# neofytr/LLMTokenizer

Measured on AMD Instinct MI355X. Metric: corpus MB/s per merge iter (train), 1 GiB synthetic corpus, higher is better.
Workload: dtype u32

## Files before the change

include/bpe_gpu.h:

```cpp
#ifndef BPE_GPU_H
#define BPE_GPU_H

#include <stddef.h>
#include <stdint.h>

#ifdef __cplusplus
extern "C" {
#endif

enum {
    BPE_GPU_OK = 0,
    BPE_GPU_EINVAL = -1,
    BPE_GPU_EHIP = -2,
    BPE_GPU_ENOMEM = -3,
    BPE_GPU_ENODEV = -4,
    BPE_GPU_ESTATE = -5,
    BPE_GPU_ERANGE = -6,
    BPE_GPU_EDATA = -7,
    BPE_GPU_EINTERNAL = -8,
    BPE_GPU_EIO = -9
};

typedef struct bpe_gpu_ctx bpe_gpu_ctx;

// ... 109 lines not shown
int bpe_gpu_decode_docs(bpe_gpu_ctx *ctx, const uint32_t *ids, size_t len, const uint64_t *id_off,
                        size_t ndocs, const uint32_t *pairs, size_t n_merges,
                        uint8_t *out, size_t cap, size_t *out_len, uint64_t *byte_off);
int bpe_gpu_docs_window(const uint64_t *doc_off, size_t ndocs, uint64_t n,
                        uint32_t core, uint32_t halo, uint64_t w, uint64_t *out8);

enum { BPE_SPLIT_LINES = 0, BPE_SPLIT_WORDS = 1 };
#define BPE_GPU_SPLIT_TILE 4096
#define BPE_GPU_SPLIT_GRID 2048
int bpe_gpu_split_rule(int preset, uint8_t *cls, uint16_t *brk);
int bpe_gpu_split_info(uint64_t *out4);
int bpe_gpu_split(bpe_gpu_ctx *ctx, const uint8_t *cls, const uint16_t *brk, size_t *ndocs);
int bpe_gpu_fetch_split_offsets(bpe_gpu_ctx *ctx, uint64_t *out, size_t cap, size_t *count);
int bpe_gpu_encode_split(bpe_gpu_ctx *ctx, const uint32_t *pairs, size_t n_merges);

int bpe_gpu_get_stats(bpe_gpu_ctx *ctx, bpe_gpu_stats *st);

int bpe_gpu_ids_checksum(bpe_gpu_ctx *ctx, uint64_t base, uint64_t *sum);

int bpe_gpu_device_tokens(bpe_gpu_ctx *ctx, const void **dev_tok, size_t *n);

int bpe_gpu_set_profile(bpe_gpu_ctx *ctx, int on);

int bpe_gpu_kernel_profile(bpe_gpu_ctx *ctx, const char **name, double *avg_ms,
                           double *bytes_per_launch, uint64_t *launches);

int bpe_gpu_event_profile(bpe_gpu_ctx *ctx, double *avg_ms, uint64_t *launches);

#define BPE_GPU_P2P_HANDLE_BYTES 64
#define BPE_GPU_P2P_MAX_RANKS 16
// ... 35 lines not shown
```

llmtokenizer_amd/_lib.py:

```python
import atexit
import ctypes
import os

HERE = os.path.dirname(os.path.abspath(__file__))
LIB_PATH = os.environ.get("BPE_LIB") or os.path.join(HERE, "libbpe_amd.so")

EXPORTS = [
    "get_file", "dump_pairs", "read_pairs", "print_text", "print_graph", "compress",
    "decompress", "render_pairs", "resolve_pair", "is_less",
    "dyn_arr_create", "dyn_arr_free", "dyn_arr_set", "dyn_arr_append", "dyn_arr_get",
    "dyn_arr_sort", "dyn_arr_max", "dyn_arr_min",
    "hash_table_create", "hash_table_destroy", "hash_table_insert", "hash_table_delete",
    "hash_table_search", "hash_table_clear", "hash_table_merge",
    "compress_ex", "bpe_train_bytes", "bpe_encode_bytes", "bpe_last_stats",
    "bpe_train_bytes_devices", "compress_multi", "bpe_release_engines", "bpe_encode_docs", "bpe_decode_docs",
    "bpe_encode_split",
    "bpe_gpu_device_count", "bpe_gpu_create", "bpe_gpu_destroy", "bpe_gpu_load", "bpe_gpu_synth",
    "bpe_gpu_train", "bpe_gpu_fetch_merges", "bpe_gpu_fetch_ids", "bpe_gpu_encode", "bpe_gpu_decode",
    "bpe_gpu_get_stats", "bpe_gpu_set_merge_log", "bpe_gpu_fetch_merge_log", "bpe_gpu_device_tokens", "bpe_gpu_kernel_profile", "bpe_gpu_set_profile", "bpe_gpu_event_profile",
    "bpe_gpu_strerror",
    "bpe_gpu_last_error", "bpe_gpu_train_ex",
    "bpe_gpu_comm_id", "bpe_gpu_group_create", "bpe_gpu_group_destroy", "bpe_gpu_group_shards",
    "bpe_gpu_group_load", "bpe_gpu_group_synth", "bpe_gpu_group_train", "bpe_gpu_group_encode", "bpe_gpu_group_fetch_merges",
    "bpe_gpu_group_fetch_ids", "bpe_gpu_group_get_stats", "bpe_gpu_group_exchange_mode", "bpe_gpu_shard_halo", "bpe_gpu_group_kernel_profile",
    "bpe_gpu_group_create_p2p", "bpe_gpu_group_p2p_connect", "bpe_gpu_group_transport",
    "bpe_gpu_group_create_local_p2p", "bpe_gpu_ids_checksum", "bpe_gpu_group_ids_checksum", "bpe_gpu_load_fd",
    "bpe_gpu_fetch_ids_range", "bpe_gpu_group_fetch_ids_range", "bpe_gpu_device_pci", "bpe_gpu_peer_access",
    "bpe_gpu_fetch_events", "bpe_gpu_trim",
    "bpe_gpu_encode_docs", "bpe_gpu_fetch_doc_offsets", "bpe_gpu_docs_info", "bpe_gpu_decode_docs",
    "bpe_gpu_docs_window",
    "bpe_gpu_split_rule", "bpe_gpu_split_info", "bpe_gpu_split", "bpe_gpu_fetch_split_offsets", "bpe_gpu_encode_split",
]


class GpuStats(ctypes.Structure):
    _fields_ = [(n, ctypes.c_uint64) for n in (
        "n_in", "n_out", "merges", "iterations", "distinct_pairs", "merged_buckets",
        "tracked_iters", "tie_events", "edge_events", "rule_ties", "table_grows", "keys")] + \
        [(n, ctypes.c_double) for n in ("ms_init", "ms_train", "ms_total", "ms_count_pass")] + \
        [(n, ctypes.c_uint64) for n in ("candidates", "occurrences", "l1_rescanned", "spec_hits", "spec_misses",
                                                     "count_pass_span", "hot_rebuilds", "hot_mode", "hot_scanned",
                                                     "enc_path", "enc_windows", "relists", "batches",
                                                     "batch_dropped", "batch_retries", "table_updates")] + \
        [(n, ctypes.c_double) for n in ("ms_scan_span", "ms_apply_span")] + \
        [(n, ctypes.c_uint64) for n in ("track_exact", "track_skipped", "track_violations", "track_light")] + \
        [(n, ctypes.c_uint64) for n in ("end_list", "end_count", "end_skipgate", "end_dup", "end_tie", "end_conflict",
# ... 120 lines not shown
    L.bpe_gpu_fetch_doc_offsets.argtypes = [vp, vp, sz, ctypes.POINTER(sz)]
    L.bpe_gpu_docs_info.argtypes = [vp, vp]
    L.bpe_gpu_decode_docs.argtypes = [vp, vp, sz, vp, sz, vp, sz, vp, sz, ctypes.POINTER(sz), vp]
    L.bpe_gpu_docs_window.argtypes = [vp, sz, ctypes.c_uint64, ctypes.c_uint32, ctypes.c_uint32, ctypes.c_uint64, vp]
    L.bpe_encode_docs.argtypes = [vp, sz, vp, sz, ctypes.POINTER(DynArr), ctypes.c_int, ctypes.POINTER(sz),
                                  ctypes.POINTER(u64p)]
    L.bpe_encode_docs.restype = u32p
    L.bpe_decode_docs.argtypes = [vp, sz, vp, sz, ctypes.POINTER(DynArr), ctypes.c_int, ctypes.POINTER(sz),
                                  ctypes.POINTER(u64p)]
    L.bpe_decode_docs.restype = ctypes.c_void_p
    L.bpe_gpu_split_rule.argtypes = [ctypes.c_int, vp, vp]
    L.bpe_gpu_split_info.argtypes = [vp]
    L.bpe_gpu_split.argtypes = [vp, vp, vp, ctypes.POINTER(sz)]
    L.bpe_gpu_fetch_split_offsets.argtypes = [vp, vp, sz, ctypes.POINTER(sz)]
    L.bpe_gpu_encode_split.argtypes = [vp, vp, sz]
    L.bpe_encode_split.argtypes = [vp, sz, vp, vp, ctypes.POINTER(DynArr), ctypes.c_int, ctypes.POINTER(sz),
                                   ctypes.POINTER(u64p), ctypes.POINTER(u64p), ctypes.POINTER(sz)]
    L.bpe_encode_split.restype = u32p
    L.bpe_release_engines.argtypes = []
    L.bpe_release_engines.restype = None
    _LIB = L
    atexit.register(L.bpe_release_engines)
    return L


def check(rc, what):
    if rc != 0:
        L = load()
        raise BpeError(f"{what}: {L.bpe_gpu_strerror(rc).decode()} ({L.bpe_gpu_last_error().decode()})")
```

llmtokenizer_amd/api.py:

```python
import ctypes
import os
import weakref

import numpy as np

from . import _lib
from ._lib import BpeError, GpuStats

_u32p = ctypes.POINTER(ctypes.c_uint32)


def _arr_to_merges(arr_p):
    L = _lib.load()
    last = arr_p.contents.last_index
    k = max(0, last - 255)
    out = np.zeros((k, 2), dtype=np.uint32)
    buf = (ctypes.c_uint32 * 2)()
    for r in range(k):
        if not L.dyn_arr_get(arr_p, 256 + r, ctypes.cast(buf, ctypes.c_void_p)):
            raise BpeError(f"merge list has no record for id {256 + r}")
        out[r] = (buf[0], buf[1])
    return out


# ... 129 lines not shown
def split_rule(preset):
    if preset not in SPLIT_PRESETS:
        raise BpeError(f"split_rule: no preset {preset!r} (have {sorted(SPLIT_PRESETS)})")
    L = _lib.load()
    cls = np.zeros(256, dtype=np.uint8)
    brk = np.zeros(16, dtype=np.uint16)
    _lib.check(L.bpe_gpu_split_rule(SPLIT_PRESETS[preset], cls.ctypes.data_as(ctypes.c_void_p),
                                    brk.ctypes.data_as(ctypes.c_void_p)), "split_rule")
    return cls, brk


def split_info():
    out = np.zeros(4, dtype=np.uint64)
    _lib.check(_lib.load().bpe_gpu_split_info(out.ctypes.data_as(ctypes.c_void_p)), "split_info")
    return {"tile": int(out[0]), "grid_bytes": int(out[1])}


def _rule_tables(rule):
    cls, brk = split_rule(rule) if isinstance(rule, str) else rule
    cls = np.ascontiguousarray(cls, dtype=np.uint8).reshape(-1)
    brk = np.ascontiguousarray(brk, dtype=np.uint16).reshape(-1)
    if cls.size != 256 or brk.size != 16:
        raise BpeError("split rule: cls must hold 256 entries and brk 16")
    return cls, brk


def encode_split(data: bytes, merges, rule="words", device=0):
    L = _lib.load()
    cls, brk = _rule_tables(rule)
    buf = np.frombuffer(data, dtype=np.uint8)
# ... 433 lines not shown
```

llmtokenizer_amd/csrc/batch.hip:

```cpp
#pragma once
#include "engine_common.h"

namespace bpeamd {

static_assert(TOPK == 64, "a wave holds a list, one entry per lane");
static_assert(BRB == 2 * (1024 / 64), "the select's 16 waves merge two partial lists each");
#ifndef BPE_SU
#define BPE_SU 1
#endif
#ifndef BPE_FORM_PRINT
#define BPE_FORM_PRINT 0
#endif
#ifndef BPE_RU
#define BPE_RU 4
#endif
#ifndef BPE_AU
#define BPE_AU 1
#endif
constexpr uint32_t AU = BPE_AU;
constexpr uint32_t SU = BPE_SU;
#ifndef BPE_RUN_THREAD_PAIRS
#define BPE_RUN_THREAD_PAIRS 16
#endif
constexpr uint32_t RUN_THREAD_PAIRS = BPE_RUN_THREAD_PAIRS, RUN_Q = 256;
// ... 29 lines not shown
        const uint32_t c = (uint32_t)__popcll(lo);
        if (r >= c) {
            r -= c;
            M >>= w;
            pos += w;
        } else {
            M = lo;
        }
    }
    return pos;
}

enum { BT_SCAN_IN = 0, BT_SCAN_CAND, BT_SCAN_OUT, BT_APPLY_IN, BT_APPLY_PRO, BT_APPLY_A, BT_APPLY_B, BT_SEL_IN,
       BT_SEL_RED, BT_SEL_LIST, BT_SEL_OUT, BT_SEL_FORMED, BT_SEL_CAND, BT_SEL_FOLD, BT_SEL_WB,
       BT_F_TIE, BT_F_CM, BT_F_MEMB, BT_F_FOLD, BT_F_PRE, BT_F_CHK, BT_B_DEC, BT_B_UPD, BT_R_LOAD, BT_R_SORT, BT_R_TREE, BT_N };
static_assert(BT_N <= TS_N, "batch stamps fit a timeline row");
__device__ inline uint32_t bat_idx(const Eng *E) {
    return E->dbgts ? (uint32_t)(E->bat->nbatch + E->bat->nretry) : 0u;
}

struct KV {
    unsigned long long v, k;
};
__device__ __attribute__((always_inline)) inline KV kv_empty() { return KV{0ull, ~0ull}; }
__device__ __attribute__((always_inline)) inline bool kv_ahead(const KV &x, const KV &y) { return x.v > y.v || (x.v == y.v && x.k < y.k); }
__device__ __attribute__((always_inline)) inline KV kv_shfl(const KV &x, int src) { return KV{__shfl(x.v, src), __shfl(x.k, src)}; }
__device__ __attribute__((always_inline)) inline KV kv_xor(const KV &x, int m) { return KV{__shfl_xor(x.v, m), __shfl_xor(x.k, m)}; }

__device__ __attribute__((always_inline)) inline KV wave_sort64(KV x) {
    const uint32_t lane = lane_id();
#pragma unroll
// ... 583 lines not shown
            prev = kv_shfl(ep, 63);
            __builtin_amdgcn_fence(__ATOMIC_RELEASE, "wavefront");
            __builtin_amdgcn_wave_barrier();
            if (!more) break;
        }
    }
    }
    uint32_t k = kk;
    if (tid < 64 && stop == STOP_NONE) {
        ts_mark(E, bi, BT_SEL_FORMED, false);
#if BPE_FORM_PRINT
        if (E->dbg_form && md + 1 >= E->dbg_form && lane == 0)
            printf("form shard %u md %u passes %u k %u end %u why %u skipped %u D %llu B %llu pend %u zrate %u\n", E->shard,
                   md, npass, kk, kend, endwhy, nskt, D, (unsigned long long)Bsz, tpend, B->zrate);
#endif
        uint32_t mode[NBK], off[NBK], len[NBK], tl[NBK], slot[NBK], slot_k[NBK], nb[NBK], bpre[NBK];
        unsigned long long pre[NBK];
#pragma unroll
        for (uint32_t b = 0; b < NBK; b++) {
            const uint32_t q = 64 * b + lane;
            mode[b] = 1;
            off[b] = len[b] = tl[b] = 0;
            if (q < k) {
                const uint32_t mu = fm_u[q], mv = fm_v[q];
                cand_of(E, mu, mv, true, srank, E->poff, &mode[b], &off[b], &len[b]);
                const uint32_t tlu = E->tlen[mu], tlv = E->tlen[mv];
                tl[b] = tlu + tlv;
                Bg->mla[q] = tlu;
                Bg->mlb[q] = tlv;
                Bg->nskb[q] = (uint8_t)fm_nsk[q];
                Bg->cnew[q] = 0;
// ... 15 lines not shown
            why_end = 7;
        }
        const unsigned long long pcut = sh && ovm < k ? bank_shfl(pre, ovm - 1) : 0ull;
        unsigned long long sumlen = 0;
#pragma unroll
        for (uint32_t b = 0; b < NBK; b++) {
            const uint32_t q = 64 * b + lane;
            slot_k[b] = slot[b];
            if (sh && q >= ovm) len[b] = slot_k[b] = 0;
            if (sh && ovm < k && q >= ovm) pre[b] = pcut;
            sumlen += q < k ? len[b] : 0u;
        }
        const unsigned long long stage_end = bank_shfl(pre, k - 1);
        sumlen = wave_sum(sumlen);
        uint32_t wk[NBK];
        unsigned long long sumw = 0, big = 0;
#pragma unroll
        for (uint32_t b = 0; b < NBK; b++) {
            const uint32_t q = 64 * b + lane;
            wk[b] = q < k && mode[b] != 0 && E->scan_occd ? min(len[b], fm_c[q] + len[b] / E->scan_occd) : len[b];
            sumw += q < k ? wk[b] : 0u;
        }
        sumw = wave_sum(sumw);
#pragma unroll
        for (uint32_t b = 0; b < NBK; b++) {
            const uint32_t q = 64 * b + lane;
            nb[b] = q < k ? 1 + (uint32_t)(sumw ? (uint64_t)(BSB - k) * wk[b] / sumw : 0) : 0;
            bpre[b] = nb[b];
            if (q < k) big = max(big, ((unsigned long long)wk[b] << 8) | (255u - q));
        }
        bank_scan(bpre);
        for (int o = 32; o > 0; o >>= 1) big = max(big, (unsigned long long)__shfl_xor(big, o));
        const uint32_t used = bank_shfl(bpre, k - 1);
        const uint32_t bigm = 255u - (uint32_t)(big & 255u);
        const uint32_t extra = BSB - used;
#pragma unroll
        for (uint32_t b = 0; b < NBK; b++) {
            const uint32_t q = 64 * b + lane;
            if (q < k) {
                B->a[q] = fm_u[q];
                B->b[q] = fm_v[q];
                B->cnt[q] = fm_c[q];
                B->mode[q] = mode[b];
                B->off[q] = off[b];
                B->len[q] = len[b];
                B->sbase[q] = (uint32_t)(pre[b] - slot_k[b]);
                B->R[q] = 0;
                B->bound[q] = 0;
                B->blk0[q] = bpre[b] - nb[b] + (q > bigm ? extra : 0);
                B->tmask[q] = (uint8_t)fm_tm[q];
                B->tspan[q] = (uint32_t)min(fm_span[q], 0xFFFFFFFFull);
                ctl[q] = tl[b];
            }
        }
        const uint32_t nsk = k ? fm_nsk[k - 1] : 0u;
        if (lane == 0) {
            B->sbase[k] = (uint32_t)stage_end;
            B->blk0[k] = BSB;
            B->sumlen = (uint32_t)sumlen;
            B->over = ovm < k ? ovm : BK;
            B->tpend = tpend < k ? tpend : BK;
            Bg->nsk = nsk;
            Bg->gr_n = 0;
#pragma unroll
            for (uint32_t g = 0; g < GRUN; g++) {
                Bg->gr_tk[g] = 0;
                Bg->gr_endc[g] = 0xFFFFFFFFu;
                Bg->gr_ready[g] = 0;
            }
            B->ztot = 0;
            B->tbar = 0;
            B->tlog_n = 0;
            B->why[why_end]++;
// ... 547 lines not shown
            }
#pragma unroll
            for (uint32_t bb = 0; bb < NBK; bb++) {
                unsigned long long tm = tadj.w[bb];
                for (int o = 32; o > 0; o >>= 1) tm |= __shfl_xor(tm, o);
                if (lane == 0 && tm) atomicOr(&B->adj[mg][bb], tm);
            }
        }
    }
}

template <bool SH>
__global__ __launch_bounds__(SCAN_T) void k_bscan(const Eng *__restrict__ E, const Ctl *__restrict__ C) {
    if (C->stop) return;
    Bat *B = E->bat;
    const uint32_t bi = bat_idx(E);
    ts_mark(E, bi, BT_SCAN_IN, true);
    if (threadIdx.x == 0) atomicMax(&B->sc_in, ~wall_clock64());
    __shared__ uint32_t s[4][DENSE];
    __shared__ uint32_t list[SCAN_T * SU * FR];
    __shared__ uint16_t ltag[SCAN_T * SU * FR];
    __shared__ uint32_t lcount, gbase, list_n, covc, sm, sk, sz0, bRs;
    __shared__ uint32_t lr_n, lr_brk, lr_pos[RUN_Q];
    __shared__ unsigned long long badj[NBK];
    __shared__ uint32_t gcnt[2];
    __shared__ uint32_t sa[BK], sb[BK];
    __shared__ RoleTab rt;
    __shared__ BHalo H;
    __shared__ uint32_t wmx[2][16];
    const uint32_t tid = threadIdx.x;
    const uint32_t sgen = ((uint32_t)(B->nbatch + B->nretry) & 0x0FFFFFFFu) + 1u;
    if (tid == 0) {
        sm = BK;
        covc = lcount = bRs = 0;
        lr_n = 0;
#pragma unroll
        for (uint32_t b = 0; b < NBK; b++) badj[b] = 0;
        gcnt[0] = gcnt[1] = 0;
        sk = B->k;
        sz0 = B->z0;
    }
    for (uint32_t q = tid; q < RH; q += SCAN_T) {
        rt.id[q] = HOLE;
        rt.fl[q] = 0;
    }
    for (uint32_t q = tid; q < RP; q += SCAN_T) rt.pk[q] = 0;
    uint32_t mla = 0;
    if (tid < BK) {
        const uint32_t lo = B->blk0[tid], hi = B->blk0[tid + 1];
        const uint32_t ma = B->a[tid];
        sa[tid] = ma;
        sb[tid] = B->b[tid];
        mla = E->tlen[ma];
        if (blockIdx.x >= lo && blockIdx.x < hi && tid < B->k) sm = tid;
    }
    __syncthreads();
    const uint32_t k = sk, m = sm, z0 = sz0;
    if (m >= k) {
        if (tid == 0) atomicMax(&B->sc_out, wall_clock64());
        return;
    }
    MK tadj = mk_zero();
    if (tid < k) {
        rt.put(sa[tid], sb[tid], mla, tid);
        if (SH) {
            Halo h;
            shard_halo(E->erec, E->nshards, E->shard, sa[tid], &h);
            H.hlr[tid] = h.hlrun;
            H.myi[tid] = h.myidx;
            if (tid == 0)
                for (int q = 0; q < 3; q++) {
                    H.HL[q] = h.HL[q];
                    H.HR[q] = h.HR[q];
                }
        }
    }
    const uint32_t a = sa[m], b = sb[m], z = z0 + m;
    const uint32_t la = E->tlen[a], lb = E->tlen[b];
    const uint32_t mode = B->mode[m], off = B->off[m], len = B->len[m];
    const uint32_t bid = blockIdx.x - B->blk0[m], nblk = B->blk0[m + 1] - B->blk0[m];
    const uint32_t sbase = B->sbase[m];
    uint32_t *occz = E->ids_out + sbase;
    uint16_t *tagz = E->btag + sbase;
    const uint32_t sslice = B->sbase[m + 1] - sbase;
#define STG(IDX, WHERE) if ((IDX) >= sslice) { B->ra_err = 12; } else
    uint32_t *Rm = &B->R[m];
    const int64_t n = (int64_t)E->n0;
    const uint32_t *__restrict__ tok = E->tok;
    const uint32_t want = mode == 2 ? a : b;
    const uint32_t lim = min(DENSE, z0 + k);
    for (uint32_t v = 0; v < 4; v++)
        for (uint32_t x = tid; x < lim; x += SCAN_T) s[v][x] = 0;
    __syncthreads();
    auto tok_at = [&](int64_t p) -> uint32_t { return tok_at_b<SH>(tok, H, p, n); };

    if (a != b) {
        static_assert(SU == 1 && BPE_WFLUSH, "the wave-driven candidate loop: one entry per lane per round");
        const uint32_t stride = nblk * SCAN_T;
        const uint32_t lane = tid & 63, wbase = (tid >> 6) * 64 * FR;
        uint32_t wcnt = 0, wocc = 0;
        uint32_t nent[SU];
        uint16_t ntg[SU];
        uint32_t eS = bid * SCAN_T + (tid & ~63u);
        auto load1 = [&](uint32_t s0, uint32_t &en, uint16_t &tg) {
            const uint32_t e = s0 + lane;
            en = 0;
            tg = 0xFFFFu;
            if (e < len) {
                en = mode == 0 ? E->plist[off + e] : E->occ[off + e];
                if (mode) tg = E->occnb[off + e];
            }
        };
        uint32_t pent = 0;
        uint16_t ptg = 0xFFFFu;
        auto advance = [&]() {
            eS += stride;
            if (SCAN_PD > 1) {
                nent[0] = pent;
// ... 12 lines not shown
            for (uint32_t q = lane; q < wcnt; q += 64) {
                STG(g + q, "wflush") {
                occz[g + q] = list[wbase + q];
                tagz[g + q] = ltag[wbase + q];
                }
            }
            wocc += wcnt;
            wcnt = 0;
            __builtin_amdgcn_wave_barrier();
        };
        const bool cmp = mode != 0 && E->scan_compact != 0;
        const uint32_t tsh = mode == 2 ? 8u : 0u;
        uint32_t qpos = 0, qn = 0;
        load1(eS, nent[0], ntg[0]);
        if (SCAN_PD > 1) load1(eS + stride, pent, ptg);
        for (;;) {
            uint32_t ent[SU];
            uint16_t etg[SU];
            bool val[SU];
            if (!cmp) {
                if (eS >= len) break;
                val[0] = eS + lane < len;
                ent[0] = nent[0];
                etg[0] = ntg[0];
                advance();
            } else {
                while (eS < len) {
                    const bool pass = eS + lane < len && tag_ok(((uint32_t)ntg[0] >> tsh) & 0xFFu, want);
                    const unsigned long long M = __ballot(pass);
                    const uint32_t np = (uint32_t)__popcll(M);
                    if (qn + np > 64) break;
                    const uint32_t r = lane - qn;
                    const bool mine = lane >= qn && r < np;
                    const uint32_t pv = (uint32_t)__shfl((int)nent[0], (int)(mine ? kth_bit(M, r) : lane));
                    if (mine) qpos = pv;
                    qn += np;
                    advance();
                }
                if (qn == 0) break;
                val[0] = lane < qn;
                ent[0] = qpos;
                etg[0] = 0xFFFFu;
                qn = 0;
            }
            int64_t ii[SU], jj[SU];
            TokWin W[SU];
#pragma unroll
            for (uint32_t u = 0; u < SU; u++) {
                if (mode == 2) {
                    val[u] = val[u] && tag_ok(etg[u] >> 8, want);
                    jj[u] = ent[u];
                    ii[u] = 0;
                    if (val[u]) W[u] = tok_window(tok, jj[u]);
                } else {
                    val[u] = val[u] && (mode == 0 || tag_ok(etg[u] & 0xFFu, want));
                    ii[u] = ent[u];
                    jj[u] = ii[u] + la;
                    if (val[u]) W[u] = tok_window(tok, ii[u]);
                }
            }
            bool ok[SU];
// ... 62 lines not shown
                    }
                }
                const unsigned long long om = __ballot(ok[u]);
                if (ok[u]) {
                    const uint32_t slot = wbase + wcnt + (uint32_t)__popcll(om & ((1ull << lane) - 1ull));
                    list[slot] = (uint32_t)i;
                    ltag[slot] = nb_tag(lfin, rfin);
                }
                wcnt += (uint32_t)__popcll(om);
            }
            if (wcnt + 64 > 64 * FR) flush();
        }
        if (wcnt) flush();
        if (lane == 0 && wocc) atomicAdd(&bRs, wocc);
    } else {
        for (uint32_t e0 = bid * SCAN_T; e0 < len; e0 += nblk * SCAN_T) {
            const uint32_t e = e0 + tid;
            int64_t i = 0;
            bool ok = false;
            if (e >= len) {
            } else if (mode == 2) {
                const int64_t j = E->occ[off + e];
                if (tag_ok(E->occnb[off + e] >> 8, want) && tok[j] == b) {
                    i = v_left<SH>(tok, j);
                    ok = i >= 0 && tok[i] == a;
                }
            } else {
                i = (mode == 0) ? E->plist[off + e] : E->occ[off + e];
                ok = (mode == 0 || tag_ok(E->occnb[off + e] & 0xFFu, want)) && tok[i] == a && i + la < n &&
                     tok[i + la] == b;
            }
// ... 63 lines not shown
                const uint32_t c = min(lcount, SCAN_T * SU);
                gbase = c ? atomicAdd(Rm, c) : 0u;
                bRs += c;
                lcount = 0;
                list_n = c;
            }
            __syncthreads();
            for (uint32_t q = tid; q < list_n; q += SCAN_T) {
                STG(gbase + q, "tflush") {
                occz[gbase + q] = list[q];
                tagz[gbase + q] = ltag[q];
                }
            }
            __syncthreads();
        }
        const uint32_t lane = tid & 63, wv = tid >> 6, nlr = min(lr_n, RUN_Q);
        auto segs = [&](int64_t c, uint32_t o, auto Uc, auto &&live) -> bool {
            constexpr uint32_t U = decltype(Uc)::value;
            const int64_t L0 = (n - c + la - 1) / la;
            auto posl = [&](int64_t l) -> int64_t { return l < L0 ? c + l * la : n + (l - L0); };
            int64_t P[U];
            uint32_t t[U], tx[U], f[U];
#pragma unroll
            for (uint32_t u = 0; u < U; u++) {
                const int64_t ou = (int64_t)o + 64 * u;
                P[u] = posl(ou + lane);
                t[u] = tok_at(P[u]);
                tx[u] = lane < 2 ? tok_at(posl(ou + 64 + lane)) : HOLE;
            }
            uint32_t fb = U;
#pragma unroll
// ... 57 lines not shown
                    segs(c, 64 * RUN_BU * wv, std::integral_constant<uint32_t, RUN_BU>{}, [&](uint32_t fb) {
                        if (lane == 0 && fb < RUN_BU) atomicMin(&lr_brk, wv * RUN_BU + fb);
                        __syncthreads();
                        const uint32_t gb = lr_brk, w0 = wv * RUN_BU;
                        return gb < w0 ? 0u : min(RUN_BU, gb - w0 + 1);
                    });
                    const bool done = lr_brk < NS;
                    __syncthreads();
                    if (done) break;
                    c += (int64_t)NS * 64 * la;
                }
            }
        }
    }
    __syncthreads();
    if (!SH && E->grflag) bscan_long_runs(E, B, tok, rt, H, n, z0, sgen);
    ts_mark(E, bi, BT_SCAN_CAND, false, true);
    if (tid < SKMAX && tid < B->nsk && ((B->sk_cm[tid][m >> 6] >> (m & 63)) & 1ull)) {
        const uint32_t xs = B->sk_a[tid], ys = B->sk_b[tid];
        uint32_t d = 0;
        if (xs == b && ys < lim) d += s[V_DR][ys];
        if (ys == a && xs < lim) d += s[V_DL][xs];
        if (d) atomicAdd(SH ? &E->xbat[BK + tid] : &B->sdec[tid], d);
    }
    const uint32_t Wx = xbat_vw(z0 + k);
    uint32_t *xm = SH ? E->xbat + XBH + (uint64_t)m * xbat_member_words(Wx) : nullptr;
    if (SH && blockIdx.x == 0 && tid == 0) {
        uint32_t xlm = BK;
        const int64_t F1 = C->F1, L1 = C->L1;
        const uint32_t over = B->over;
        if (F1 < n) {
            const uint32_t tf = tok[F1], tl1 = tok[L1];
            for (uint32_t mm = 0; mm < k; mm++)
                if (H.HL[0] == sa[mm] && tf == sb[mm] && (sa[mm] != sb[mm] || (H.hlr[mm] & 1))) {
                    xlm = mm;
                    break;
                }
            for (uint32_t mm = 0; mm < k && mm < over; mm++) {
                if (!(tl1 == sa[mm] && H.HR[0] == sb[mm] && (sa[mm] != sb[mm] || !(H.myi[mm] & 1)))) continue;
                uint32_t *xo = E->xbat + XBH + (uint64_t)mm * xbat_member_words(Wx);
                const uint32_t zz = z0 + mm;
// ... 17 lines not shown
                    if (st < BK) rfin = z0 + st;
                    xadd(E, xo, Wx, mm, V_DR, q);
                    xadd(E, xo, Wx, mm, V_IR, rfin);
                }
                (void)zz;
                const uint32_t g = atomicAdd(&B->R[mm], 1u);
                E->ids_out[B->sbase[mm] + g] = (uint32_t)L1;
                E->btag[B->sbase[mm] + g] = nb_tag(lfin, rfin);
                atomicAdd(&xo[0], 1u);
                atomicAdd(&xo[1], bnd);
                break;
            }
        }
        B->xl_m = xlm;
        if (over < k) atomicAdd(&E->xbat[over], 1u);
    }
    if (k > 1) {
#pragma unroll
        for (uint32_t bb = 0; bb < NBK; bb++) {
            unsigned long long t = tadj.w[bb];
            for (int o = 32; o > 0; o >>= 1) t |= __shfl_xor(t, o);
            if ((tid & 63) == 0 && t) atomicOr(&badj[bb], t);
        }
        __syncthreads();
        if (tid < NBK && badj[tid]) atomicOr(&B->adj[m][tid], badj[tid]);
    }
    uint32_t *rep = SH ? xm + 2 : E->bvecd + (uint64_t)(m * BREPL + bid % BREPL) * 4 * DENSE;
    const uint32_t vstride = SH ? Wx : DENSE;
    uint32_t mxl = 0, mxr = 0;
    for (uint32_t v = 0; v < 4; v++)
        for (uint32_t x = tid; x < lim; x += SCAN_T) {
            const uint32_t c = s[v][x];
            if (c) atomicAdd(&rep[v * vstride + x], c);
            if (v == V_DL) mxl = max(mxl, c);
            if (v == V_DR) mxr = max(mxr, c);
        }
    if (SH && tid == 0 && bRs) atomicAdd(&xm[0], bRs);
    if (k > 1) {
        for (int o = 32; o > 0; o >>= 1) {
            mxl = max(mxl, (uint32_t)__shfl_xor(mxl, o));
            mxr = max(mxr, (uint32_t)__shfl_xor(mxr, o));
        }
        if ((tid & 63) == 0) {
            wmx[0][tid >> 6] = mxl;
            wmx[1][tid >> 6] = mxr;
        }
        __syncthreads();
        if (tid == 0) {
            uint32_t l = 0, r = 0;
            for (uint32_t q = 0; q < SCAN_T / 64; q++) {
                l = max(l, wmx[0][q]);
                r = max(r, wmx[1][q]);
            }
            atomicAdd(SH ? &xm[1] : &B->bound[m], max(l + gcnt[V_DL] + covc, r + gcnt[V_DR]));
        }
    }
    ts_mark(E, bi, BT_SCAN_OUT, false, true);
    asm volatile("s_waitcnt vmcnt(0)" ::: "memory");
    __syncthreads();
    if (tid == 0) atomicMax(&B->sc_out, wall_clock64());
}
template __global__ void k_bscan<false>(const Eng *, const Ctl *);
template __global__ void k_bscan<true>(const Eng *, const Ctl *);

constexpr uint32_t XSP_SHIFT = 23;
static_assert(4 * BK < (1u << (32 - XSP_SHIFT)), "member-vector index fits above the id");
__global__ __launch_bounds__(256) void k_bpack(const Eng *__restrict__ E, const Ctl *__restrict__ C) {
    if (C->stop) return;
    const Bat *B = E->bat;
    __shared__ uint32_t pre[BK * 4 + 1];
// ... 660 lines not shown
```

llmtokenizer_amd/csrc/engine.hip:

```cpp
#include <hip/hip_runtime.h>
#include <fcntl.h>
#include <unistd.h>
#include <cerrno>

#include <algorithm>
#include <chrono>
#include <cstdio>
#include <cstdlib>
#include <cstring>
#include <string>
#include <thread>
#include <vector>
#include <unordered_map>

#include <rocprim/rocprim.hpp>

#include "../../include/bpe_gpu.h"
#include "kernels.hip"
#include "batch.hip"
#include "encode.hip"
#include "encode_win.hip"
#include "encode_docs.hip"
#include "split.hip"

// ... 1418 lines not shown
        const unsigned long long *r = &t[(size_t)b * TS_N];
        bool ok = true;
        for (int k = 0; k < BT_N; k++) ok = ok && r[k] != 0;
        if (!ok) continue;
        const double t0 = (double)~r[BT_SCAN_IN];
        for (int k = 0; k < BT_N; k++) {
            const bool in = k == BT_SCAN_IN || k == BT_APPLY_IN || k == BT_SEL_IN;
            sum[k] += ((in ? (double)~r[k] : (double)r[k]) - t0) * 1000.0 / khz;
        }
        n++;
        const unsigned long long *q = &t[(size_t)(b + 1) * TS_N];
        if (q[BT_SCAN_IN]) {
            gap += ((double)~q[BT_SCAN_IN] - (double)r[BT_SEL_OUT]) * 1000.0 / khz;
            ng++;
        }
    }
    if (!n) return;
    fprintf(stderr, "batch timeline over %u batches (us from k_bscan's first block entry):", n);
    for (int k = 1; k < BT_N; k++) fprintf(stderr, " %s %.2f;", nm[k], sum[k] / n);
    fprintf(stderr, " sel out -> next scan in %.2f\n", ng ? gap / ng : 0.0);
}

int batch_stats(bpe_gpu_ctx *c) {
    if (!c->h.bat) return 0;
    Bat hb;
    HIPCHK(hipMemcpy(&hb, c->h.bat, offsetof(Bat, pv), hipMemcpyDeviceToHost));
    c->stats.batches = hb.nbatch;
    c->stats.batch_dropped = hb.ndrop;
    c->stats.batch_retries = hb.nretry;
    c->stats.table_updates = hb.nupd;
// ... 1571 lines not shown
                 : b >= '\t' && b <= '\r'                                      ? 4
                                                                               : 0;
    for (int p = 0; p < 5; p++) brk[p] = (uint16_t)(0x1F & ~(1 << p));
    brk[3] = 1 << 4;
    return 0;
}

int bpe_gpu_split_info(uint64_t *out4) {
    if (!out4) return BPE_GPU_EINVAL;
    out4[0] = SP_TILE;
    out4[1] = (uint64_t)SP_TILE * SP_GRID;
    out4[2] = out4[3] = 0;
    return 0;
}

int bpe_gpu_split(bpe_gpu_ctx *c, const uint8_t *cls, const uint16_t *brk, size_t *ndocs) {
    if (!c || !cls || !brk || !ndocs) return BPE_GPU_EINVAL;
    if (!c->loaded) return fail(BPE_GPU_ESTATE, "split before load");
    SplitRule R;
    for (int b = 0; b < 256; b++)
        if ((R.cls[b] = cls[b]) > 15) return fail(BPE_GPU_EINVAL, "split: a class above 15");
    memcpy(R.brk, brk, sizeof R.brk);
    HIPCHK(hipSetDevice(c->dev));
    c->split_ready = false;
    const uint64_t n = c->n0, ntiles = (n + SP_TILE - 1) / SP_TILE, nwt = ntiles * (SP_T / 64);
    unsigned long long total = 0;
    uint16_t *mask = nullptr;
    unsigned long long *woff = nullptr;
    int r;
    if (n) {
// ... 107 lines not shown
```

llmtokenizer_amd/csrc/engine_common.h:

```cpp
#pragma once
#include <hip/hip_runtime.h>
#include <stddef.h>
#include <stdint.h>

namespace bpeamd {

constexpr uint32_t HOLE = 0xFFFFFFFFu;
constexpr uint32_t END_FLAG = 0x80000000u;
constexpr uint32_t MARKV = 0xFFFFFFFEu;
constexpr uint64_t END_MAX = 0x7FFFFFFDull;
__host__ __device__ inline bool is_id(uint32_t v) { return v < END_FLAG; }
__host__ __device__ inline uint32_t end_code(uint64_t d) { return END_FLAG | (uint32_t)d; }
#ifndef BPE_DENSE
#define BPE_DENSE 8192
#endif
constexpr uint32_t DENSE = BPE_DENSE;
#ifndef BPE_REPL
#define BPE_REPL 8
#endif
constexpr uint32_t REPL = BPE_REPL;
constexpr uint32_t NTHR = 16;
constexpr uint64_t CHUNK = 65536;
constexpr uint64_t DYN_LIMIT = CHUNK * NTHR;
constexpr uint64_t TRACK_LIMIT = 2 * DYN_LIMIT;
constexpr uint64_t TRACK_MIN_N = 4096;
constexpr uint64_t MERGED_B0 = 65536;
constexpr uint64_t THREAD_B0 = 256;
constexpr uint32_t L1W = 1024;
constexpr uint32_t L2W = 256;
constexpr uint32_t EDGE_WORDS = 16;
constexpr uint32_t TS_SLOTS = 16384;
enum { TS_K1_IN = 0, TS_K1_RESCAN, TS_K1_SCAN, TS_K2_IN, TS_K2_SELECT, TS_K2_APPLY_A, TS_K2_APPLY_B, TS_K1_LASTIN,
       TS_S_CAND, TS_S_LIST, TS_S_DELTA, TS_B_DVAL, TS_B_TABLE, TS_B_MARKS, TS_B_PROBE, TS_B_COUNT, TS_K1_CLEARED,
       TS_SPARE0, TS_SPARE1, TS_SPARE2, TS_SPARE3, TS_SPARE4, TS_SPARE5, TS_SPARE6, TS_SPARE7, TS_SPARE8, TS_N };

enum { V_DL = 0, V_DR = 1, V_IL = 2, V_IR = 3 };

enum : uint32_t {
    STOP_NONE = 0,
    STOP_DONE = 1,
    STOP_CAP = 2,
    STOP_EVENT = 3,
    STOP_GROW = 4,
    STOP_ERROR = 5,
    STOP_ENC_END = 6,
    STOP_MODE = 7,
    STOP_REDO = 8,
    STOP_HOT = 9,
    STOP_RELIST = 10,
// ... 35 lines not shown
constexpr uint32_t TOPK = 64;
#ifndef BPE_BK
#define BPE_BK 127
#endif
constexpr uint32_t BK = BPE_BK;
constexpr uint32_t NBK = (BK + 1) / 64;
static_assert(BK + 1 == 64 * NBK && NBK >= 1 && NBK <= 2, "BK is 63 or 127");
constexpr uint32_t SKMAX = BK;
#ifndef BPE_NLIST
#define BPE_NLIST 4
#endif
constexpr uint32_t NLIST = BPE_NLIST;
constexpr uint32_t BRB = 32;
constexpr uint32_t BREPL = 2;
constexpr uint32_t BSB = 256;
constexpr uint32_t STALL_LIMIT = 64;
constexpr uint32_t GRUN = 4;
constexpr uint32_t GR_CH = 16384;
constexpr uint32_t GR_PROBE = 4096;
__host__ __device__ inline uint64_t gr_stride(uint64_t n0) { return n0 / GR_CH + 2; }
constexpr uint32_t P2P_MAXR_B = 16;

struct Bat {
    uint32_t k, z0, applied, jstar;
    uint32_t ticket, retry, sumlen, rhold;
    unsigned long long dD;
    unsigned long long nbatch, ndrop, nretry;
    unsigned long long why[8];
    uint32_t drop_test;
    uint32_t skgate;
    unsigned long long stage_cap;
    unsigned long long sc_in, sc_out, ap_in, ap_out, sc_ticks, ap_ticks, nspan, nupd;
    uint32_t a[BK], b[BK], cnt[BK], mode[BK], off[BK], len[BK];
    uint32_t blk0[BK + 1];
    uint32_t sbase[BK + 1];
    uint32_t R[BK];
    uint32_t bound[BK];
    uint32_t Rg[BK];
    uint32_t over;
    uint32_t xl_m;
    uint32_t tpend;
    uint32_t ztot;
    uint32_t tbar, zrate;
    unsigned long long ntie, ntfail, nzero;
    uint8_t tmask[BK + 1];
    uint32_t tspan[BK];
    uint32_t tlog_n;
    unsigned long long pv[BRB * TOPK], pk[BRB * TOPK];
    uint32_t ra_k, ra_top, ra_done, ra_err;
// ... 323 lines not shown
```

Measured before the change: 118.7 million.

## Split batch scan work across blocks by weighted granules instead of whole merges

The old scheme gave each batched merge a whole number of k_bscan blocks, sized by its share of the weight plus leftovers assigned to the largest merge. The new scheme takes a prefix sum of per-merge weights and cuts the global weighted range into equal slices of 1024-entry granules, so one block can cover the tail of one merge and the head of later ones. The scan body now loops over those pieces with per-piece reset and flush of the shared histograms. The intent is to balance load across the 256 blocks and avoid a single overloaded block. The cost is more flushes and syncthreads per block, plus extra debug busy-time counters and a host-side test API.

```diff
diff --git a/include/bpe_gpu.h b/include/bpe_gpu.h
--- a/include/bpe_gpu.h
+++ b/include/bpe_gpu.h
@@ -147,6 +147,9 @@
 int bpe_gpu_fetch_split_offsets(bpe_gpu_ctx *ctx, uint64_t *out, size_t cap, size_t *count);
 int bpe_gpu_encode_split(bpe_gpu_ctx *ctx, const uint32_t *pairs, size_t n_merges);
 
+int bpe_gpu_scan_split(const uint32_t *weight, const uint32_t *len, uint32_t k, uint32_t nblk, uint32_t block,
+                       uint32_t *pieces, size_t cap, size_t *count);
+
 int bpe_gpu_get_stats(bpe_gpu_ctx *ctx, bpe_gpu_stats *st);
 
 int bpe_gpu_ids_checksum(bpe_gpu_ctx *ctx, uint64_t base, uint64_t *sum);
diff --git a/llmtokenizer_amd/_lib.py b/llmtokenizer_amd/_lib.py
--- a/llmtokenizer_amd/_lib.py
+++ b/llmtokenizer_amd/_lib.py
@@ -30,6 +30,7 @@
     "bpe_gpu_encode_docs", "bpe_gpu_fetch_doc_offsets", "bpe_gpu_docs_info", "bpe_gpu_decode_docs",
     "bpe_gpu_docs_window",
     "bpe_gpu_split_rule", "bpe_gpu_split_info", "bpe_gpu_split", "bpe_gpu_fetch_split_offsets", "bpe_gpu_encode_split",
+    "bpe_gpu_scan_split",
 ]
 
 
@@ -180,6 +181,7 @@
     L.bpe_gpu_split.argtypes = [vp, vp, vp, ctypes.POINTER(sz)]
     L.bpe_gpu_fetch_split_offsets.argtypes = [vp, vp, sz, ctypes.POINTER(sz)]
     L.bpe_gpu_encode_split.argtypes = [vp, vp, sz]
+    L.bpe_gpu_scan_split.argtypes = [vp, vp, ctypes.c_uint32, ctypes.c_uint32, ctypes.c_uint32, vp, sz, ctypes.POINTER(sz)]
     L.bpe_encode_split.argtypes = [vp, sz, vp, vp, ctypes.POINTER(DynArr), ctypes.c_int, ctypes.POINTER(sz),
                                    ctypes.POINTER(u64p), ctypes.POINTER(u64p), ctypes.POINTER(sz)]
     L.bpe_encode_split.restype = u32p
diff --git a/llmtokenizer_amd/api.py b/llmtokenizer_amd/api.py
--- a/llmtokenizer_amd/api.py
+++ b/llmtokenizer_amd/api.py
@@ -167,6 +167,19 @@
     out = np.zeros(4, dtype=np.uint64)
     _lib.check(_lib.load().bpe_gpu_split_info(out.ctypes.data_as(ctypes.c_void_p)), "split_info")
     return {"tile": int(out[0]), "grid_bytes": int(out[1])}
+
+
+def scan_split(weight, length, nblk, block):
+    w = np.ascontiguousarray(weight, dtype=np.uint32).reshape(-1)
+    n = np.ascontiguousarray(length, dtype=np.uint32).reshape(-1)
+    if w.size != n.size:
+        raise BpeError("scan_split: one weight per list")
+    out = np.zeros((max(1, w.size), 3), dtype=np.uint32)
+    cnt = ctypes.c_size_t(0)
+    _lib.check(_lib.load().bpe_gpu_scan_split(w.ctypes.data_as(ctypes.c_void_p), n.ctypes.data_as(ctypes.c_void_p),
+                                              w.size, nblk, block, out.ctypes.data_as(ctypes.c_void_p),
+                                              out.shape[0], ctypes.byref(cnt)), "scan_split")
+    return [tuple(int(x) for x in row) for row in out[:cnt.value]]
 
 
 def _rule_tables(rule):
diff --git a/llmtokenizer_amd/csrc/batch.hip b/llmtokenizer_amd/csrc/batch.hip
--- a/llmtokenizer_amd/csrc/batch.hip
+++ b/llmtokenizer_amd/csrc/batch.hip
@@ -67,7 +67,9 @@
 enum { BT_SCAN_IN = 0, BT_SCAN_CAND, BT_SCAN_OUT, BT_APPLY_IN, BT_APPLY_PRO, BT_APPLY_A, BT_APPLY_B, BT_SEL_IN,
        BT_SEL_RED, BT_SEL_LIST, BT_SEL_OUT, BT_SEL_FORMED, BT_SEL_CAND, BT_SEL_FOLD, BT_SEL_WB,
        BT_F_TIE, BT_F_CM, BT_F_MEMB, BT_F_FOLD, BT_F_PRE, BT_F_CHK, BT_B_DEC, BT_B_UPD, BT_R_LOAD, BT_R_SORT, BT_R_TREE, BT_N };
-static_assert(BT_N <= TS_N, "batch stamps fit a timeline row");
+enum { BT_X_BUSY_SUM = TS_X0, BT_X_BUSY_MAX = TS_X1, BT_X_BUSY_N = TS_X2 };
+static_assert(BT_N <= TS_X0, "batch stamps fit a timeline row");
+static_assert(SCAN_GRAN == 1024, "a granule is one round of a k_bscan block");
 __device__ inline uint32_t bat_idx(const Eng *E) {
     return E->dbgts ? (uint32_t)(E->bat->nbatch + E->bat->nretry) : 0u;
 }
@@ -681,7 +683,7 @@
             printf("form shard %u md %u passes %u k %u end %u why %u skipped %u D %llu B %llu pend %u zrate %u\n", E->shard,
                    md, npass, kk, kend, endwhy, nskt, D, (unsigned long long)Bsz, tpend, B->zrate);
 #endif
-        uint32_t mode[NBK], off[NBK], len[NBK], tl[NBK], slot[NBK], slot_k[NBK], nb[NBK], bpre[NBK];
+        uint32_t mode[NBK], off[NBK], len[NBK], tl[NBK], slot[NBK], slot_k[NBK], wpre[NBK];
         unsigned long long pre[NBK];
 #pragma unroll
         for (uint32_t b = 0; b < NBK; b++) {
@@ -727,26 +729,14 @@
         const unsigned long long stage_end = bank_shfl(pre, k - 1);
         sumlen = wave_sum(sumlen);
         uint32_t wk[NBK];
-        unsigned long long sumw = 0, big = 0;
 #pragma unroll
         for (uint32_t b = 0; b < NBK; b++) {
             const uint32_t q = 64 * b + lane;
             wk[b] = q < k && mode[b] != 0 && E->scan_occd ? min(len[b], fm_c[q] + len[b] / E->scan_occd) : len[b];
-            sumw += q < k ? wk[b] : 0u;
-        }
-        sumw = wave_sum(sumw);
-#pragma unroll
-        for (uint32_t b = 0; b < NBK; b++) {
-            const uint32_t q = 64 * b + lane;
-            nb[b] = q < k ? 1 + (uint32_t)(sumw ? (uint64_t)(BSB - k) * wk[b] / sumw : 0) : 0;
-            bpre[b] = nb[b];
-            if (q < k) big = max(big, ((unsigned long long)wk[b] << 8) | (255u - q));
-        }
-        bank_scan(bpre);
-        for (int o = 32; o > 0; o >>= 1) big = max(big, (unsigned long long)__shfl_xor(big, o));
-        const uint32_t used = bank_shfl(bpre, k - 1);
-        const uint32_t bigm = 255u - (uint32_t)(big & 255u);
-        const uint32_t extra = BSB - used;
+            wk[b] = q < k ? wk[b] : 0u;
+            wpre[b] = wk[b];
+        }
+        bank_scan(wpre);
 #pragma unroll
         for (uint32_t b = 0; b < NBK; b++) {
             const uint32_t q = 64 * b + lane;
@@ -760,16 +750,17 @@
                 B->sbase[q] = (uint32_t)(pre[b] - slot_k[b]);
                 B->R[q] = 0;
                 B->bound[q] = 0;
-                B->blk0[q] = bpre[b] - nb[b] + (q > bigm ? extra : 0);
+                B->wpre[q] = wpre[b] - wk[b];
                 B->tmask[q] = (uint8_t)fm_tm[q];
                 B->tspan[q] = (uint32_t)min(fm_span[q], 0xFFFFFFFFull);
                 ctl[q] = tl[b];
             }
         }
+        const uint32_t wsum = bank_shfl(wpre, k - 1);
         const uint32_t nsk = k ? fm_nsk[k - 1] : 0u;
         if (lane == 0) {
             B->sbase[k] = (uint32_t)stage_end;
-            B->blk0[k] = BSB;
+            B->wpre[k] = wsum;
             B->sumlen = (uint32_t)sumlen;
             B->over = ovm < k ? ovm : BK;
             B->tpend = tpend < k ? tpend : BK;
@@ -1347,13 +1338,15 @@
 __global__ __launch_bounds__(SCAN_T) void k_bscan(const Eng *__restrict__ E, const Ctl *__restrict__ C) {
     if (C->stop) return;
     Bat *B = E->bat;
-    const uint32_t bi = bat_idx(E);
+    const uint32_t bi = uni(bat_idx(E));
     ts_mark(E, bi, BT_SCAN_IN, true);
     if (threadIdx.x == 0) atomicMax(&B->sc_in, ~wall_clock64());
     __shared__ uint32_t s[4][DENSE];
     __shared__ uint32_t list[SCAN_T * SU * FR];
     __shared__ uint16_t ltag[SCAN_T * SU * FR];
-    __shared__ uint32_t lcount, gbase, list_n, covc, sm, sk, sz0, bRs;
+    __shared__ uint32_t lcount, gbase, list_n, covc, sk, sz0, bRs;
+    __shared__ uint32_t pq0, pq1, plo0, phi1;
+    __shared__ unsigned long long t_in;
     __shared__ uint32_t lr_n, lr_brk, lr_pos[RUN_Q];
     __shared__ unsigned long long badj[NBK];
     __shared__ uint32_t gcnt[2];
@@ -1361,17 +1354,15 @@
     __shared__ RoleTab rt;
     __shared__ BHalo H;
     __shared__ uint32_t wmx[2][16];
-    const uint32_t tid = threadIdx.x;
-    const uint32_t sgen = ((uint32_t)(B->nbatch + B->nretry) & 0x0FFFFFFFu) + 1u;
+    uint32_t tid = threadIdx.x;
+    const uint32_t sgen = uni(((uint32_t)(B->nbatch + B->nretry) & 0x0FFFFFFFu) + 1u);
     if (tid == 0) {
-        sm = BK;
-        covc = lcount = bRs = 0;
-        lr_n = 0;
-#pragma unroll
-        for (uint32_t b = 0; b < NBK; b++) badj[b] = 0;
-        gcnt[0] = gcnt[1] = 0;
+        pq0 = BK;
+        pq1 = 0;
+        lcount = 0;
         sk = B->k;
         sz0 = B->z0;
+        if (E->dbgts) t_in = wall_clock64();
     }
     for (uint32_t q = tid; q < RH; q += SCAN_T) {
         rt.id[q] = HOLE;
@@ -1379,21 +1370,31 @@
     }
     for (uint32_t q = tid; q < RP; q += SCAN_T) rt.pk[q] = 0;
     uint32_t mla = 0;
+    uint32_t mlo = 0, mhi = 0;
+    __syncthreads();
     if (tid < BK) {
-        const uint32_t lo = B->blk0[tid], hi = B->blk0[tid + 1];
         const uint32_t ma = B->a[tid];
         sa[tid] = ma;
         sb[tid] = B->b[tid];
         mla = E->tlen[ma];
-        if (blockIdx.x >= lo && blockIdx.x < hi && tid < B->k) sm = tid;
+        if (tid < B->k) {
+            scan_split_piece(B->wpre, B->len, B->k, BSB, blockIdx.x, tid, &mlo, &mhi);
+            if (mlo < mhi) {
+                atomicMin(&pq0, tid);
+                atomicMax(&pq1, tid);
+            }
+        }
     }
     __syncthreads();
-    const uint32_t k = sk, m = sm, z0 = sz0;
-    if (m >= k) {
+    const uint32_t k = uni(sk), z0 = uni(sz0);
+    if (k == 0) {
         if (tid == 0) atomicMax(&B->sc_out, wall_clock64());
         return;
     }
-    MK tadj = mk_zero();
+    if (mlo < mhi) {
+        if (tid == pq0) plo0 = mlo;
+        if (tid == pq1) phi1 = mhi;
+    }
     if (tid < k) {
         rt.put(sa[tid], sb[tid], mla, tid);
         if (SH) {
@@ -1408,33 +1409,50 @@
                 }
         }
     }
-    const uint32_t a = sa[m], b = sb[m], z = z0 + m;
+    const int64_t n = (int64_t)E->n0;
+    const uint32_t *__restrict__ tok = E->tok;
+    const uint32_t lim = min(DENSE, z0 + k);
+    const uint32_t Wx = xbat_vw(z0 + k);
+    auto tok_at = [&](int64_t p) -> uint32_t { return tok_at_b<SH>(tok, H, p, n); };
+    __syncthreads();
+    const uint32_t q0 = uni(pq0), q1 = uni(pq1);
+    for (uint32_t m = q0; m <= q1; m++) {
+    const uint32_t e_lo = m == q0 ? uni(plo0) : 0u, e_hi = m == q1 ? uni(phi1) : B->len[m];
+    if (e_lo >= e_hi) continue;
+    asm volatile("" : "+v"(tid));
+    __syncthreads();
+    if (tid == 0) {
+        uint32_t zero = 0;
+        asm volatile("" : "+v"(zero));
+        covc = bRs = zero;
+        lr_n = zero;
+#pragma unroll
+        for (uint32_t bb = 0; bb < NBK; bb++) badj[bb] = zero;
+        gcnt[0] = gcnt[1] = zero;
+    }
+    MK tadj = mk_zero();
+    const uint32_t a = uni(sa[m]), b = uni(sb[m]), z = z0 + m;
     const uint32_t la = E->tlen[a], lb = E->tlen[b];
-    const uint32_t mode = B->mode[m], off = B->off[m], len = B->len[m];
-    const uint32_t bid = blockIdx.x - B->blk0[m], nblk = B->blk0[m + 1] - B->blk0[m];
+    const uint32_t mode = B->mode[m], off = B->off[m] + e_lo, len = e_hi - e_lo;
     const uint32_t sbase = B->sbase[m];
     uint32_t *occz = E->ids_out + sbase;
     uint16_t *tagz = E->btag + sbase;
     const uint32_t sslice = B->sbase[m + 1] - sbase;
 #define STG(IDX, WHERE) if ((IDX) >= sslice) { B->ra_err = 12; } else
     uint32_t *Rm = &B->R[m];
-    const int64_t n = (int64_t)E->n0;
-    const uint32_t *__restrict__ tok = E->tok;
     const uint32_t want = mode == 2 ? a : b;
-    const uint32_t lim = min(DENSE, z0 + k);
     for (uint32_t v = 0; v < 4; v++)
         for (uint32_t x = tid; x < lim; x += SCAN_T) s[v][x] = 0;
     __syncthreads();
-    auto tok_at = [&](int64_t p) -> uint32_t { return tok_at_b<SH>(tok, H, p, n); };
 
     if (a != b) {
         static_assert(SU == 1 && BPE_WFLUSH, "the wave-driven candidate loop: one entry per lane per round");
-        const uint32_t stride = nblk * SCAN_T;
+        const uint32_t stride = SCAN_T;
         const uint32_t lane = tid & 63, wbase = (tid >> 6) * 64 * FR;
         uint32_t wcnt = 0, wocc = 0;
         uint32_t nent[SU];
         uint16_t ntg[SU];
-        uint32_t eS = bid * SCAN_T + (tid & ~63u);
+        uint32_t eS = tid & ~63u;
         auto load1 = [&](uint32_t s0, uint32_t &en, uint16_t &tg) {
             const uint32_t e = s0 + lane;
             en = 0;
@@ -1477,6 +1495,7 @@
         uint32_t qpos = 0, qn = 0;
         load1(eS, nent[0], ntg[0]);
         if (SCAN_PD > 1) load1(eS + stride, pent, ptg);
+        TokWin W[SU] = {};
         for (;;) {
             uint32_t ent[SU];
             uint16_t etg[SU];
@@ -1507,7 +1526,6 @@
                 qn = 0;
             }
             int64_t ii[SU], jj[SU];
-            TokWin W[SU];
 #pragma unroll
             for (uint32_t u = 0; u < SU; u++) {
                 if (mode == 2) {
@@ -1600,7 +1618,7 @@
         if (wcnt) flush();
         if (lane == 0 && wocc) atomicAdd(&bRs, wocc);
     } else {
-        for (uint32_t e0 = bid * SCAN_T; e0 < len; e0 += nblk * SCAN_T) {
+        for (uint32_t e0 = 0; e0 < len; e0 += SCAN_T) {
             const uint32_t e = e0 + tid;
             int64_t i = 0;
             bool ok = false;
@@ -1694,7 +1712,7 @@
             }
             __syncthreads();
         }
-        const uint32_t lane = tid & 63, wv = tid >> 6, nlr = min(lr_n, RUN_Q);
+        const uint32_t lane = tid & 63, wv = uni(tid >> 6), nlr = min(lr_n, RUN_Q);
         auto segs = [&](int64_t c, uint32_t o, auto Uc, auto &&live) -> bool {
             constexpr uint32_t U = decltype(Uc)::value;
             const int64_t L0 = (n - c + la - 1) / la;
@@ -1782,8 +1800,6 @@
         }
     }
     __syncthreads();
-    if (!SH && E->grflag) bscan_long_runs(E, B, tok, rt, H, n, z0, sgen);
-    ts_mark(E, bi, BT_SCAN_CAND, false, true);
     if (tid < SKMAX && tid < B->nsk && ((B->sk_cm[tid][m >> 6] >> (m & 63)) & 1ull)) {
         const uint32_t xs = B->sk_a[tid], ys = B->sk_b[tid];
         uint32_t d = 0;
@@ -1791,8 +1807,59 @@
         if (ys == a && xs < lim) d += s[V_DL][xs];
         if (d) atomicAdd(SH ? &E->xbat[BK + tid] : &B->sdec[tid], d);
     }
-    const uint32_t Wx = xbat_vw(z0 + k);
     uint32_t *xm = SH ? E->xbat + XBH + (uint64_t)m * xbat_member_words(Wx) : nullptr;
+    if (k > 1) {
+#pragma unroll
+        for (uint32_t bb = 0; bb < NBK; bb++) {
+            unsigned long long t = tadj.w[bb];
+            for (int o = 32; o > 0; o >>= 1) t |= __shfl_xor(t, o);
+            if ((tid & 63) == 0 && t) atomicOr(&badj[bb], t);
+        }
+        __syncthreads();
+        if (tid < NBK && badj[tid]) atomicOr(&B->adj[m][tid], badj[tid]);
+    }
+    uint32_t *rep = SH ? xm + 2 : E->bvecd + (uint64_t)(m * BREPL + blockIdx.x % BREPL) * 4 * DENSE;
+    const uint32_t vstride = SH ? Wx : DENSE;
+    uint32_t mxl = 0, mxr = 0;
+    for (uint32_t v = 0; v < 4; v++)
+        for (uint32_t x = tid; x < lim; x += SCAN_T) {
+            const uint32_t c = s[v][x];
+            if (c) atomicAdd(&rep[v * vstride + x], c);
+            if (v == V_DL) mxl = max(mxl, c);
+            if (v == V_DR) mxr = max(mxr, c);
+        }
+    if (SH && tid == 0 && bRs) atomicAdd(&xm[0], bRs);
+    if (k > 1) {
+        for (int o = 32; o > 0; o >>= 1) {
+            mxl = max(mxl, (uint32_t)__shfl_xor(mxl, o));
+            mxr = max(mxr, (uint32_t)__shfl_xor(mxr, o));
+        }
+        if ((tid & 63) == 0) {
+            wmx[0][tid >> 6] = mxl;
+            wmx[1][tid >> 6] = mxr;
+        }
+        __syncthreads();
+        if (tid == 0) {
+            uint32_t l = 0, r = 0;
+            for (uint32_t q = 0; q < SCAN_T / 64; q++) {
+                l = max(l, wmx[0][q]);
+                r = max(r, wmx[1][q]);
+            }
+            atomicAdd(SH ? &xm[1] : &B->bound[m], max(l + gcnt[V_DL] + covc, r + gcnt[V_DR]));
+        }
+    }
+    }
+#undef STG
+    __syncthreads();
+    if (!SH && E->grflag) bscan_long_runs(E, B, tok, rt, H, n, z0, sgen);
+    ts_mark(E, bi, BT_SCAN_CAND, false, true);
+    if (E->dbgts && tid == 0 && q0 <= q1) {
+        unsigned long long *row = &E->dbgts[(uint64_t)(bi % TS_SLOTS) * TS_N];
+        const unsigned long long busy = wall_clock64() - t_in;
+        atomicAdd(&row[BT_X_BUSY_SUM], busy);
+        atomicMax(&row[BT_X_BUSY_MAX], busy);
+        atomicAdd(&row[BT_X_BUSY_N], 1ull);
+    }
     if (SH && blockIdx.x == 0 && tid == 0) {
         uint32_t xlm = BK;
         const int64_t F1 = C->F1, L1 = C->L1;
@@ -1840,46 +1907,6 @@
         }
         B->xl_m = xlm;
         if (over < k) atomicAdd(&E->xbat[over], 1u);
-    }
-    if (k > 1) {
-#pragma unroll
-        for (uint32_t bb = 0; bb < NBK; bb++) {
-            unsigned long long t = tadj.w[bb];
-            for (int o = 32; o > 0; o >>= 1) t |= __shfl_xor(t, o);
-            if ((tid & 63) == 0 && t) atomicOr(&badj[bb], t);
-        }
-        __syncthreads();
-        if (tid < NBK && badj[tid]) atomicOr(&B->adj[m][tid], badj[tid]);
-    }
-    uint32_t *rep = SH ? xm + 2 : E->bvecd + (uint64_t)(m * BREPL + bid % BREPL) * 4 * DENSE;
-    const uint32_t vstride = SH ? Wx : DENSE;
-    uint32_t mxl = 0, mxr = 0;
-    for (uint32_t v = 0; v < 4; v++)
-        for (uint32_t x = tid; x < lim; x += SCAN_T) {
-            const uint32_t c = s[v][x];
-            if (c) atomicAdd(&rep[v * vstride + x], c);
-            if (v == V_DL) mxl = max(mxl, c);
-            if (v == V_DR) mxr = max(mxr, c);
-        }
-    if (SH && tid == 0 && bRs) atomicAdd(&xm[0], bRs);
-    if (k > 1) {
-        for (int o = 32; o > 0; o >>= 1) {
-            mxl = max(mxl, (uint32_t)__shfl_xor(mxl, o));
-            mxr = max(mxr, (uint32_t)__shfl_xor(mxr, o));
-        }
-        if ((tid & 63) == 0) {
-            wmx[0][tid >> 6] = mxl;
-            wmx[1][tid >> 6] = mxr;
-        }
-        __syncthreads();
-        if (tid == 0) {
-            uint32_t l = 0, r = 0;
-            for (uint32_t q = 0; q < SCAN_T / 64; q++) {
-                l = max(l, wmx[0][q]);
-                r = max(r, wmx[1][q]);
-            }
-            atomicAdd(SH ? &xm[1] : &B->bound[m], max(l + gcnt[V_DL] + covc, r + gcnt[V_DR]));
-        }
     }
     ts_mark(E, bi, BT_SCAN_OUT, false, true);
     asm volatile("s_waitcnt vmcnt(0)" ::: "memory");
diff --git a/llmtokenizer_amd/csrc/engine.hip b/llmtokenizer_amd/csrc/engine.hip
--- a/llmtokenizer_amd/csrc/engine.hip
+++ b/llmtokenizer_amd/csrc/engine.hip
@@ -1456,6 +1456,26 @@
             gap += ((double)~q[BT_SCAN_IN] - (double)r[BT_SEL_OUT]) * 1000.0 / khz;
             ng++;
         }
+    }
+    {
+        double rsum = 0, rmax = 0, bsum = 0, msum = 0;
+        uint32_t nr = 0;
+        for (uint64_t b = 1; b + 1 < nb && b < TS_SLOTS; b++) {
+            const unsigned long long *r = &t[(size_t)b * TS_N];
+            if (!r[BT_X_BUSY_N] || !r[BT_X_BUSY_SUM]) continue;
+            const double mean = (double)r[BT_X_BUSY_SUM] / (double)r[BT_X_BUSY_N], ratio = (double)r[BT_X_BUSY_MAX] / mean;
+            fprintf(stderr, "scan split: batch %llu blocks %llu busiest %.2f us mean %.2f us ratio %.3f\n",
+                    (unsigned long long)b, r[BT_X_BUSY_N], (double)r[BT_X_BUSY_MAX] * 1000.0 / khz, mean * 1000.0 / khz, ratio);
+            rsum += ratio;
+            rmax = std::max(rmax, ratio);
+            bsum += (double)r[BT_X_BUSY_MAX] * 1000.0 / khz;
+            msum += mean * 1000.0 / khz;
+            nr++;
+        }
+        if (nr)
+            fprintf(stderr, "scan split over %u batches: busiest / mean block %.3f on average, %.3f at most; busiest %.2f us, "
+                    "mean %.2f us per batch (sum of busiest / sum of means %.3f)\n", nr, rsum / nr, rmax, bsum / nr,
+                    msum / nr, bsum / msum);
     }
     if (!n) return;
     fprintf(stderr, "batch timeline over %u batches (us from k_bscan's first block entry):", n);
@@ -3057,6 +3077,40 @@
     return 0;
 }
 
+int bpe_gpu_scan_split(const uint32_t *weight, const uint32_t *len, uint32_t k, uint32_t nblk, uint32_t block,
+                       uint32_t *pieces, size_t cap, size_t *count) {
+    if (!weight || !len || !count || k > BK || !nblk || nblk > BSB || block >= nblk) return BPE_GPU_EINVAL;
+    uint32_t wpre[BK + 1];
+    uint64_t tot = 0;
+    for (uint32_t q = 0; q < k; q++) {
+        wpre[q] = (uint32_t)tot;
+        tot += weight[q];
+    }
+    if (tot >> 32) return BPE_GPU_EINVAL;
+    wpre[k] = (uint32_t)tot;
+    uint32_t q0 = BK, q1 = 0, lo0 = 0, hi1 = 0;
+    for (uint32_t q = 0; q < k; q++) {
+        uint32_t lo, hi;
+        scan_split_piece(wpre, len, k, nblk, block, q, &lo, &hi);
+        if (lo >= hi) continue;
+        if (q < q0) q0 = q, lo0 = lo;
+        if (q >= q1) q1 = q, hi1 = hi;
+    }
+    size_t np = 0;
+    for (uint32_t m = q0; m <= q1 && m < k; m++) {
+        const uint32_t e_lo = m == q0 ? lo0 : 0u, e_hi = m == q1 ? hi1 : len[m];
+        if (e_lo >= e_hi) continue;
+        if (pieces && np < cap) {
+            pieces[3 * np] = m;
+            pieces[3 * np + 1] = e_lo;
+            pieces[3 * np + 2] = e_hi;
+        }
+        np++;
+    }
+    *count = np;
+    return pieces && np > cap ? BPE_GPU_EINVAL : 0;
+}
+
 int bpe_gpu_split(bpe_gpu_ctx *c, const uint8_t *cls, const uint16_t *brk, size_t *ndocs) {
     if (!c || !cls || !brk || !ndocs) return BPE_GPU_EINVAL;
     if (!c->loaded) return fail(BPE_GPU_ESTATE, "split before load");
diff --git a/llmtokenizer_amd/csrc/engine_common.h b/llmtokenizer_amd/csrc/engine_common.h
--- a/llmtokenizer_amd/csrc/engine_common.h
+++ b/llmtokenizer_amd/csrc/engine_common.h
@@ -32,7 +32,8 @@
 constexpr uint32_t TS_SLOTS = 16384;
 enum { TS_K1_IN = 0, TS_K1_RESCAN, TS_K1_SCAN, TS_K2_IN, TS_K2_SELECT, TS_K2_APPLY_A, TS_K2_APPLY_B, TS_K1_LASTIN,
        TS_S_CAND, TS_S_LIST, TS_S_DELTA, TS_B_DVAL, TS_B_TABLE, TS_B_MARKS, TS_B_PROBE, TS_B_COUNT, TS_K1_CLEARED,
-       TS_SPARE0, TS_SPARE1, TS_SPARE2, TS_SPARE3, TS_SPARE4, TS_SPARE5, TS_SPARE6, TS_SPARE7, TS_SPARE8, TS_N };
+       TS_SPARE0, TS_SPARE1, TS_SPARE2, TS_SPARE3, TS_SPARE4, TS_SPARE5, TS_SPARE6, TS_SPARE7, TS_SPARE8,
+       TS_X0, TS_X1, TS_X2, TS_N };
 
 enum { V_DL = 0, V_DR = 1, V_IL = 2, V_IR = 3 };
 
@@ -98,6 +99,27 @@
 constexpr uint32_t BRB = 32;
 constexpr uint32_t BREPL = 2;
 constexpr uint32_t BSB = 256;
+constexpr uint32_t SCAN_GRAN = 1024;
+__host__ __device__ inline uint32_t scan_granules(uint32_t len) { return len / SCAN_GRAN + (len % SCAN_GRAN != 0); }
+__host__ __device__ inline uint32_t scan_split_first(uint64_t P, uint32_t w, uint32_t g, uint64_t T, uint32_t nblk,
+                                                     uint32_t b) {
+    if (b >= nblk) return g;
+    const uint64_t cut = (uint64_t)b * T, at = (uint64_t)nblk * P;
+    if (cut <= at) return 0;
+    if (!w) return g;
+    const uint64_t num = (cut - at) * g, den = (uint64_t)nblk * w;
+    const uint64_t j = num / den + (num % den != 0);
+    return j < g ? (uint32_t)j : g;
+}
+__host__ __device__ inline void scan_split_piece(const uint32_t *wpre, const uint32_t *len, uint32_t k, uint32_t nblk,
+                                                 uint32_t b, uint32_t q, uint32_t *lo, uint32_t *hi) {
+    const uint32_t g = scan_granules(len[q]), w = wpre[q + 1] - wpre[q];
+    const uint32_t j0 = scan_split_first(wpre[q], w, g, wpre[k], nblk, b);
+    const uint32_t j1 = scan_split_first(wpre[q], w, g, wpre[k], nblk, b + 1);
+    const uint64_t e0 = (uint64_t)j0 * SCAN_GRAN, e1 = (uint64_t)j1 * SCAN_GRAN;
+    *lo = e0 < len[q] ? (uint32_t)e0 : len[q];
+    *hi = e1 < len[q] ? (uint32_t)e1 : len[q];
+}
 constexpr uint32_t STALL_LIMIT = 64;
 constexpr uint32_t GRUN = 4;
 constexpr uint32_t GR_CH = 16384;
@@ -116,7 +138,7 @@
     unsigned long long stage_cap;
     unsigned long long sc_in, sc_out, ap_in, ap_out, sc_ticks, ap_ticks, nspan, nupd;
     uint32_t a[BK], b[BK], cnt[BK], mode[BK], off[BK], len[BK];
-    uint32_t blk0[BK + 1];
+    uint32_t wpre[BK + 1];
     uint32_t sbase[BK + 1];
     uint32_t R[BK];
     uint32_t bound[BK];
```

Result: slower. 117.3 million (-1.2%).
